# JuliaGaussianProcesses/AugmentedGPLikelihoods.jl

Measured on AMD Instinct MI355X. Metric: CAVI sweeps/sec (N obs, M inducing) + max |Δnat-param| vs CPU ref, higher is better.
Workload: dtype f32 via f16 hi/lo split operands (3 f16 MFMA products per f32 product, f32 accumulate, f64 reductions and M x M update)

## Files before the change

augmentedgplikelihoods.jl_amd/csrc/agpl_syrk.hip:

```cpp
#include <cstdlib>

#include "agpl_common.h"

namespace {

typedef _Float16 h8 __attribute__((ext_vector_type(8)));
typedef float f32x4 __attribute__((ext_vector_type(4)));
typedef unsigned u32x4 __attribute__((ext_vector_type(4)));

constexpr int BS = 128;
constexpr int kPanel = 256;
constexpr int kStagePts = 32;
constexpr uint32_t kImageMagic = 0x41474951u;

struct AccImageHeader {
    uint32_t magic;
    int32_t scale_exp;
    float max_abs;
    uint32_t reserved;
    int64_t N;
    int32_t M;
    int32_t pad[57];
};
static_assert(sizeof(AccImageHeader) == 256, "header size");

__device__ __forceinline__ f32x4 mfma32(h8 a, h8 b, f32x4 c) {
    return __builtin_amdgcn_mfma_f32_16x16x32_f16(a, b, c, 0, 0, 0);
}

#define AGPL_E_SPLIT2(x0_, s0_, x1_, s1_, H_, L_)                                                              \
    do {                                                                                                       \
        asm("v_fma_mixlo_f16 %0, %1, %2, 0" : "=v"(H_) : "v"(x0_), "v"(s0_));                                  \
        asm("v_fma_mixhi_f16 %0, %1, %2, 0" : "+v"(H_) : "v"(x1_), "v"(s1_));                                  \
        asm("v_fma_mixlo_f16 %0, %1, %2, -%3 op_sel_hi:[0,0,1]" : "=v"(L_) : "v"(x0_), "v"(s0_), "v"(H_));     \
        asm("v_fma_mixhi_f16 %0, %1, %2, -%3 op_sel:[0,0,1] op_sel_hi:[0,0,1]"                                 \
            : "+v"(L_)                                                                                         \
            : "v"(x1_), "v"(s1_), "v"(H_));                                                                    \
    } while (0)
#define AGPL_E_GFMA(acc_, b_, x_) asm volatile("v_fmac_f32 %0, %1, %2" : "+v"(acc_) : "v"(b_), "v"(x_))
#define AGPL_Q_JOIN2(H_, L_, x0_, x1_)                                                                         \
    do {                                                                                                       \
        asm("v_fma_mix_f32 %0, %1, 1.0, %2 op_sel_hi:[1,0,1]" : "=v"(x0_) : "v"(H_), "v"(L_));                 \
        asm("v_fma_mix_f32 %0, %1, 1.0, %2 op_sel:[1,0,1] op_sel_hi:[1,0,1]" : "=v"(x1_) : "v"(H_), "v"(L_));  \
    } while (0)

__global__ __launch_bounds__(256) void absmax_kernel(int64_t n4, int ntail, const float4 *__restrict__ x, unsigned *__restrict__ out) {
    unsigned m = 0u;
    for (int64_t i = (int64_t)blockIdx.x * blockDim.x + threadIdx.x; i < n4; i += (int64_t)gridDim.x * blockDim.x) {
        const float4 v = x[i];
        m = max(m, __float_as_uint(v.x) & 0x7FFFFFFFu);
        m = max(m, __float_as_uint(v.y) & 0x7FFFFFFFu);
        m = max(m, __float_as_uint(v.z) & 0x7FFFFFFFu);
        m = max(m, __float_as_uint(v.w) & 0x7FFFFFFFu);
    }
    if (blockIdx.x == 0 && (int)threadIdx.x < ntail)
        m = max(m, __float_as_uint(reinterpret_cast<const float *>(x)[4 * n4 + threadIdx.x]) & 0x7FFFFFFFu);
#pragma unroll
    for (int o = 32; o > 0; o >>= 1) m = max(m, (unsigned)__shfl_xor((int)m, o));
    if ((threadIdx.x & 63) == 0 && m) atomicMax(out, m);
}

__global__ __launch_bounds__(256) void find_bad_kernel(int64_t n, const float *__restrict__ x, float limit,
                                                       unsigned long long *__restrict__ out) {
    for (int64_t i = (int64_t)blockIdx.x * blockDim.x + threadIdx.x; i < n; i += (int64_t)gridDim.x * blockDim.x) {
        const float a = fabsf(x[i]);
        if (!(a < limit)) atomicMin(out, (unsigned long long)i);
    }
}

__global__ __launch_bounds__(256) void accumulate_image_kernel(int64_t N, int M, int Msrc, int64_t nps, float scale, int scale_exp,
                                                               float max_abs, const float *__restrict__ Phi,
                                                               unsigned char *__restrict__ image) {
    __shared__ float tile[16][BS + 1];
    const int nb = M / BS;
    if (blockIdx.x == 0 && threadIdx.x == 0) {
        AccImageHeader *h = reinterpret_cast<AccImageHeader *>(image);
        h->magic = kImageMagic;
        h->scale_exp = scale_exp;
        h->max_abs = max_abs;
        h->reserved = 0;
        h->N = N;
        h->M = M;
    }
    h8 *blocks = reinterpret_cast<h8 *>(image + sizeof(AccImageHeader));
    const int64_t nblk = nps * nb;
    for (int64_t blk = blockIdx.x; blk < nblk; blk += gridDim.x) {
        const int64_t ps = blk / nb;
        const int fb = (int)(blk - ps * nb);
        {
            const int pt = threadIdx.x >> 4, f0 = (threadIdx.x & 15) * 8;
            const int64_t n = ps * 16 + pt;
            float4 a = {0.f, 0.f, 0.f, 0.f}, b = a;
            if (n < N) {
                const int fg = fb * BS + f0;
                const float *src = Phi + n * (int64_t)Msrc + fg;
                if (!(Msrc & 3) && fg + 8 <= Msrc) {
                    a = *reinterpret_cast<const float4 *>(src);
                    b = *reinterpret_cast<const float4 *>(src + 4);
                } else {
                    float t[8];
#pragma unroll
                    for (int j = 0; j < 8; ++j) t[j] = fg + j < Msrc ? src[j] : 0.f;
                    a = float4{t[0], t[1], t[2], t[3]};
                    b = float4{t[4], t[5], t[6], t[7]};
                }
            }
            float *d = &tile[pt][f0];
            d[0] = a.x; d[1] = a.y; d[2] = a.z; d[3] = a.w;
            d[4] = b.x; d[5] = b.y; d[6] = b.z; d[7] = b.w;
        }
        __syncthreads();
        const int plane = threadIdx.x >> 7, row = threadIdx.x & 127;
        h8 hi, lo;
#pragma unroll
        for (int j = 0; j < 8; ++j) {
            const float x = tile[plane * 8 + j][row] * scale;
            const _Float16 a = (_Float16)x;
            hi[j] = a;
            lo[j] = (_Float16)(x - (float)a);
        }
        blocks[(blk * 2 + 0) * 256 + threadIdx.x] = hi;
        blocks[(blk * 2 + 1) * 256 + threadIdx.x] = lo;
        __syncthreads();
    }
}

__global__ __launch_bounds__(256) void acc_prep_kernel(int64_t N, int64_t Npad, int L, const float *__restrict__ gamma,
                                                        const float *__restrict__ beta, float *__restrict__ gb,
                                                        unsigned *__restrict__ scal) {
    __shared__ unsigned red[2][4];
    const int64_t total = (int64_t)L * Npad;
    unsigned m = 0u, bd = 0u;
    for (int64_t i = (int64_t)blockIdx.x * blockDim.x + threadIdx.x; i < total; i += (int64_t)gridDim.x * blockDim.x) {
        const int64_t l = i / Npad, n = i - l * Npad;
        const bool in = n < N;
        const float gv = in ? gamma[l * N + n] : 0.f;
        const unsigned gbits = __float_as_uint(gv), ab = gbits & 0x7FFFFFFFu;
        const bool bad = ab >= 0x7F800000u || ((gbits >> 31) && ab != 0u);
        if (bad) bd = max(bd, (unsigned)min((int64_t)0x7FFFFFFE, l * N + n) + 1u);
        m = max(m, bad ? 0u : ab);
        float *rec = gb + (l * (Npad / 32) + n / 32) * 64 + (n & 31);
        rec[0] = gv;
        rec[32] = in ? beta[l * N + n] : 0.f;
    }
#pragma unroll
    for (int o = 32; o > 0; o >>= 1) {
        m = max(m, (unsigned)__shfl_xor((int)m, o));
        bd = max(bd, (unsigned)__shfl_xor((int)bd, o));
    }
    if ((threadIdx.x & 63) == 0) {
        red[0][threadIdx.x >> 6] = m;
        red[1][threadIdx.x >> 6] = bd;
    }
    __syncthreads();
    if (threadIdx.x == 0) {
        for (int w = 1; w < 4; ++w) {
            m = max(m, red[0][w]);
            bd = max(bd, red[1][w]);
        }
        if (m) atomicMax(scal, m);
        if (bd) atomicMax(scal + 1, bd);
    }
}

__device__ __forceinline__ int acc_scale_exp(unsigned gmax) {
    int eB = gmax ? 126 - (int)(gmax >> 23) : 0;
    return eB < -60 ? -60 : (eB > 60 ? 60 : eB);
}

#ifdef AGPL_QTRACE
__device__ unsigned long long g_qtrace[64 * 16 * 8];
constexpr bool kTrace = true;
#else
constexpr bool kTrace = false;
#endif

#ifdef AGPL_SYRK_L2PROBE
#define AGPL_PROBE_T(t_) ((t_) & 3)
#else
#define AGPL_PROBE_T(t_) (t_)
#endif
#ifdef AGPL_SYRK_NODMA
#define AGPL_PROBE_LOAD(t_) ((t_) < 3)
#else
#define AGPL_PROBE_LOAD(t_) true
#endif
#ifndef AGPL_S_PRE
#define AGPL_S_PRE 3
#endif
constexpr int kStepBytes = 32768;
constexpr int kRing = 4;
constexpr int kRecBytes = 256;
constexpr int kStripLds = kRing * kStepBytes + 8 * kRing * kRecBytes;

template <bool DIAG>
__device__ __forceinline__ void syrk_strip_body(unsigned char *smem_raw, int64_t N, int64_t Npad, int M, int nsplit, int chunk, int nbig, int small, int l,
                                                int s, int I, int J, const unsigned char *__restrict__ image,
                                                const float *__restrict__ gb_all, const unsigned *__restrict__ scal,
                                                float *__restrict__ slabG, float *__restrict__ slabg) {
    typedef __attribute__((address_space(3))) void lds_void;
    const int lane = threadIdx.x & 63;
    const int wave = __builtin_amdgcn_readfirstlane(threadIdx.x >> 6);
    const int nb = M / BS;
    const int cq0 = DIAG ? wave : 2 * wave, cq1 = DIAG ? 15 - wave : 2 * wave + 1;
    const AccImageHeader *hdr = reinterpret_cast<const AccImageHeader *>(image);
    const h8 *blocks = reinterpret_cast<const h8 *>(image + sizeof(AccImageHeader));
    const int eA = hdr->scale_exp;
    const int eB = acc_scale_exp(scal[0]);
    const float sB = __uint_as_float((unsigned)(127 + eB) << 23);

    int64_t nbeg, nend;
    agpl_slice_range(s, chunk, nbig, small, N, nbeg, nend);
    const int nstep = (int)((nend - nbeg + kStagePts - 1) / kStagePts);
    const int64_t ps0 = nbeg / 16;
    const int64_t slice_pitch = (int64_t)nb * 2 * 256;

    int ln = lane;
    asm volatile("" : "+v"(ln));
    const int kg = ln >> 4, lr = ln & 15;
    const int rbS = (wave >> 2) & 1, qd = wave & 3;
    const h8 *a_src = blocks + ((ps0 * nb + 2 * I + rbS) * 2) * 256 + qd * 64 + lane;
    const int a_dst = rbS * 2 * 4096 + qd * 1024;
    const int R0 = 32 * wave + lr;
    const h8 *b_src = blocks + (((ps0 + (kg >> 1)) * nb + 2 * J + (R0 >> 7)) * 2) * 256 + (kg & 1) * 128 + (R0 & 127);
    const float *gb_src = gb_all + ((int64_t)l * (Npad / 32) + nbeg / 32) * 64 + lane;
    float *gbuf = reinterpret_cast<float *>(smem_raw + kRing * kStepBytes + wave * kRing * kRecBytes);

    f32x4 acc[16][2];
#pragma unroll
    for (int i = 0; i < 16; ++i) acc[i][0] = acc[i][1] = f32x4{0.f, 0.f, 0.f, 0.f};
    float gacc0 = 0.f, gacc1 = 0.f;
    u32x4 rh0 = {0, 0, 0, 0}, rl0 = rh0, rh1 = rh0, rl1 = rh0;
    h8 bh0, bl0, bh1, bl1;

#define AGPL_S_DMA(t_, k_)                     \
    do {                                                                                                        \
        unsigned char *d_ = smem_raw + ((t_) & (kRing - 1)) * kStepBytes + ((k_) >> 1) * 16384 + a_dst + ((k_) & 1) * 4096; \
        const h8 *src_ = a_src + (int64_t)(2 * AGPL_PROBE_T(t_) + ((k_) >> 1)) * slice_pitch + ((k_) & 1) * 256; \
        if (AGPL_PROBE_LOAD(t_)) __builtin_amdgcn_global_load_lds(src_, (lds_void *)d_, 16, 0, 0);              \
    } while (0)
#define AGPL_S_DMAG(t_)                                                                                         \
    if (AGPL_PROBE_LOAD(t_))                                                                                    \
    __builtin_amdgcn_global_load_lds(gb_src + (int64_t)(t_) * 64, (lds_void *)(gbuf + ((t_) & (kRing - 1)) * 64), 4, 0, 0)
#define AGPL_S_LOADB(t_)                                                                                        \
    do {                                                                                                        \
        const h8 *src_ = b_src + (int64_t)(2 * AGPL_PROBE_T(t_)) * slice_pitch;                                 \
        const h8 *srcl_ = src_ + 256;  \
        if (AGPL_PROBE_LOAD(t_))                                                                                \
        asm volatile("global_load_dwordx4 %0, %4, off\n\tglobal_load_dwordx4 %1, %5, off\n\t"                   \
                     "global_load_dwordx4 %2, %4, off offset:256\n\tglobal_load_dwordx4 %3, %5, off offset:256"  \
                     : "+v"(rh0), "+v"(rl0), "+v"(rh1), "+v"(rl1)                                               \
                     : "v"(src_), "v"(srcl_)                                                                    \
                     : "memory");                                                                               \
    } while (0)
#define AGPL_S_CVT(RH_, RL_, g0_, g1_, b0_, b1_, GA_)                                                           \
    do {                                                                                                        \
        float x0_, x1_;                                                                                         \
        AGPL_Q_JOIN2(RH_, RL_, x0_, x1_);                                                                       \
        if (DIAG) {                                                                                             \
            AGPL_E_GFMA(GA_, b0_, x0_);                                                                         \
            AGPL_E_GFMA(GA_, b1_, x1_);                                                                         \
        }                                                                                                       \
        AGPL_E_SPLIT2(x0_, g0_, x1_, g1_, RH_, RL_);                                                            \
    } while (0)
#define AGPL_S_CVTQ(q_, tt_, keepf_)                                                                            \
    do {                                                                                                        \
        const float *gq_ = gbuf + ((tt_) & (kRing - 1)) * 64 + 8 * kg + 4 * ((q_) & 1);                         \
        float4 g4_ = *reinterpret_cast<const float4 *>(gq_);                                                    \
        g4_.x *= sB, g4_.y *= sB, g4_.z *= sB, g4_.w *= sB;                                                     \
        float4 b4_ = {0.f, 0.f, 0.f, 0.f};                                                                      \
        if (DIAG) {                                                                                             \
            b4_ = *reinterpret_cast<const float4 *>(gq_ + 32);                                                  \
            if (!(keepf_)) b4_ = float4{0.f, 0.f, 0.f, 0.f};                                                    \
        }                                                                                                       \
        if ((q_) == 0) {                                                                                        \
            AGPL_S_CVT(rh0.x, rl0.x, g4_.x, g4_.y, b4_.x, b4_.y, gacc0);                                        \
            AGPL_S_CVT(rh0.y, rl0.y, g4_.z, g4_.w, b4_.z, b4_.w, gacc0);                                        \
            AGPL_S_CVT(rh1.x, rl1.x, g4_.x, g4_.y, b4_.x, b4_.y, gacc1);                                        \
            AGPL_S_CVT(rh1.y, rl1.y, g4_.z, g4_.w, b4_.z, b4_.w, gacc1);                                        \
        } else {                                                                                                \
            AGPL_S_CVT(rh0.z, rl0.z, g4_.x, g4_.y, b4_.x, b4_.y, gacc0);                                        \
            AGPL_S_CVT(rh0.w, rl0.w, g4_.z, g4_.w, b4_.z, b4_.w, gacc0);                                        \
            AGPL_S_CVT(rh1.z, rl1.z, g4_.x, g4_.y, b4_.x, b4_.y, gacc1);                                        \
            AGPL_S_CVT(rh1.w, rl1.w, g4_.z, g4_.w, b4_.z, b4_.w, gacc1);                                        \
        }                                                                                                       \
    } while (0)
#define AGPL_S_TAKEB()                       \
    do {                                                                                                        \
        bh0 = __builtin_bit_cast(h8, rh0);                                                                      \
        bl0 = __builtin_bit_cast(h8, rl0);                                                                      \
        bh1 = __builtin_bit_cast(h8, rh1);                                                                      \
        bl1 = __builtin_bit_cast(h8, rl1);                                                                      \
    } while (0)

    const int fa = (kg >> 1) * 1024 + (kg & 1) * 128 + lr;
#define AGPL_S_AOFF(i_) (fa + ((i_) >> 3) * 512 + ((i_) & 7) * 16)
#define AGPL_S_LDSB(t_)                                                                                         \
    do {                                                                                                        \
        const u32x4 *sn_ = reinterpret_cast<const u32x4 *>(smem_raw + ((t_) & (kRing - 1)) * kStepBytes);       \
        rh0 = sn_[AGPL_S_AOFF(cq0)];                                                                            \
        rl0 = sn_[256 + AGPL_S_AOFF(cq0)];                                                                      \
        rh1 = sn_[AGPL_S_AOFF(cq1)];                                                                            \
        rl1 = sn_[256 + AGPL_S_AOFF(cq1)];                                                                      \
    } while (0)

#pragma unroll
    for (int t = 0; t < 3; ++t)
        if (t < nstep) {
            AGPL_S_DMAG(t);
            AGPL_S_DMA(t, 0);
            AGPL_S_DMA(t, 1);
            AGPL_S_DMA(t, 2);
            AGPL_S_DMA(t, 3);
        }
    if (!DIAG) AGPL_S_LOADB(0);
    asm volatile("s_waitcnt vmcnt(0)" ::: "memory");
    __builtin_amdgcn_sched_barrier(0);
    if (DIAG) {
        __builtin_amdgcn_s_barrier();
        AGPL_S_LDSB(0);
    }
    AGPL_S_CVTQ(0, 0, true);
    AGPL_S_CVTQ(1, 0, true);
    AGPL_S_TAKEB();
    if (!DIAG) AGPL_S_LOADB(nstep > 1 ? 1 : 0);

    [[maybe_unused]] unsigned long long q0 = 0, q1 = 0, qw = 0, qa = 0, qb = 0, qr0 = 0;
    if (kTrace) {
        q0 = __builtin_amdgcn_s_memtime();
        qr0 = __builtin_amdgcn_s_memrealtime();
    }
    for (int t = 0; t < nstep; ++t) {
        if (kTrace) qa = __builtin_amdgcn_s_memtime();
        if (!DIAG) __builtin_amdgcn_s_barrier();
        if (kTrace && !DIAG) qw += __builtin_amdgcn_s_memtime() - qa;
        const bool more = t + 1 < nstep;
        const int tl = t + 2 < nstep ? t + 2 : nstep - 1;
        const h8 *st = reinterpret_cast<const h8 *>(smem_raw + (t & (kRing - 1)) * kStepBytes);
#define AGPL_S_HOOK(h_)                                                                                         \
    do {                                                                                                        \
        if (!DIAG) {                                                                                            \
            if ((h_) < 4 && t + 3 < nstep) {                                                                    \
                if ((h_) == 0) AGPL_S_DMAG(t + 3);                                                              \
                AGPL_S_DMA(t + 3, h_);                                                                          \
            }                                                                                                   \
            if ((h_) == 5) {  \
                __builtin_amdgcn_sched_barrier(0);                                                              \
                if (kTrace) qb = __builtin_amdgcn_s_memtime();                                                  \
                if (t + 3 < nstep) asm volatile("s_waitcnt vmcnt(5)" ::: "memory");                             \
                else asm volatile("s_waitcnt vmcnt(0)" ::: "memory");                                           \
                if (kTrace) q1 += __builtin_amdgcn_s_memtime() - qb;                                            \
                __builtin_amdgcn_sched_barrier(0);                                                              \
            }                                                                                                   \
            if ((h_) == 6) AGPL_S_CVTQ(0, t + 1, more);                                                         \
            if ((h_) == 8) AGPL_S_CVTQ(1, t + 1, more);                                                         \
        } else {                                                                                                \
             \
             \
             \
                 \
            if ((h_) == 7) {                                                                                    \
                __builtin_amdgcn_sched_barrier(0);                                                              \
                if (kTrace) qb = __builtin_amdgcn_s_memtime();                                                  \
                if (t + 2 < nstep) asm volatile("s_waitcnt vmcnt(5)" ::: "memory");                             \
                else asm volatile("s_waitcnt vmcnt(0)" ::: "memory");                                           \
                if (kTrace) q1 += __builtin_amdgcn_s_memtime() - qb;                                            \
                if (kTrace) qb = __builtin_amdgcn_s_memtime();                                                  \
                __builtin_amdgcn_s_barrier();                                                                   \
                if (kTrace) qw += __builtin_amdgcn_s_memtime() - qb;                                            \
                __builtin_amdgcn_sched_barrier(0);                                                              \
                AGPL_S_LDSB(more ? t + 1 : t);                 \
            }                                                                                                   \
            if ((h_) >= 8 && (h_) < 12 && t + 3 < nstep) {                                                      \
                if ((h_) == 8) AGPL_S_DMAG(t + 3);                                                              \
                AGPL_S_DMA(t + 3, (h_) - 8);                                                                    \
            }                                                                                                   \
            if ((h_) == 9) AGPL_S_CVTQ(0, t + 1, more);                                                         \
            if ((h_) == 11) AGPL_S_CVTQ(1, t + 1, more);                                                        \
        }                                                                                                       \
    } while (0)
        h8 nbh0, nbl0, nbh1, nbl1;
        constexpr int kPre = AGPL_S_PRE;
        h8 af[kPre + 1][2];
#pragma unroll
        for (int j = 0; j < kPre; ++j) {
            af[j][0] = st[AGPL_S_AOFF(j)];
            af[j][1] = st[256 + AGPL_S_AOFF(j)];
        }
#pragma unroll
        for (int i = 0; i < 16; ++i) {
            if (!DIAG && (i == 0 || i == 12)) {
                if ((wave >= 4) == (i == 0)) __builtin_amdgcn_s_setprio(1);
                else __builtin_amdgcn_s_setprio(0);
            }
            if (i + kPre < 16) {
                af[(i + kPre) % (kPre + 1)][0] = st[AGPL_S_AOFF(i + kPre)];
                af[(i + kPre) % (kPre + 1)][1] = st[256 + AGPL_S_AOFF(i + kPre)];
            }
            if (!DIAG) {
                const h8 ahc = af[i % (kPre + 1)][0], alc = af[i % (kPre + 1)][1];
                acc[i][0] = mfma32(ahc, bh0, acc[i][0]);
                acc[i][1] = mfma32(ahc, bh1, acc[i][1]);
                acc[i][0] = mfma32(ahc, bl0, acc[i][0]);
                acc[i][1] = mfma32(ahc, bl1, acc[i][1]);
                acc[i][0] = mfma32(alc, bh0, acc[i][0]);
                acc[i][1] = mfma32(alc, bh1, acc[i][1]);
            } else {
                const h8 ahc = af[i % (kPre + 1)][0], alc = af[i % (kPre + 1)][1];
                if (i >= cq0) {
                    acc[i][0] = mfma32(ahc, bh0, acc[i][0]);
                    acc[i][0] = mfma32(ahc, bl0, acc[i][0]);
                    acc[i][0] = mfma32(alc, bh0, acc[i][0]);
                }
                if (i >= cq1) {
                    acc[i][1] = mfma32(ahc, bh1, acc[i][1]);
                    acc[i][1] = mfma32(ahc, bl1, acc[i][1]);
                    acc[i][1] = mfma32(alc, bh1, acc[i][1]);
                }
            }
            AGPL_S_HOOK(i);
            if (i == (DIAG ? 12 : 10)) {
                nbh0 = __builtin_bit_cast(h8, rh0);
                nbl0 = __builtin_bit_cast(h8, rl0);
                nbh1 = __builtin_bit_cast(h8, rh1);
                nbl1 = __builtin_bit_cast(h8, rl1);
                if (!DIAG) AGPL_S_LOADB(tl);
            }
        }
#undef AGPL_S_HOOK
        bh0 = nbh0;
        bl0 = nbl0;
        bh1 = nbh1;
        bl1 = nbl1;
    }
    if (!DIAG) __builtin_amdgcn_s_setprio(0);
#ifdef AGPL_QTRACE
    if (blockIdx.x < 64 && lane == 0) {
        unsigned long long *o = g_qtrace + ((size_t)blockIdx.x * 16 + wave) * 8;
        o[0] = q1;
        o[1] = __builtin_amdgcn_s_memtime() - q0;
        o[2] = qw;
        o[5] = __builtin_amdgcn_s_memrealtime() - qr0;
        o[6] = (unsigned long long)nstep | ((unsigned long long)(DIAG ? 1 : 0) << 32) | ((unsigned long long)cq0 << 40);
        o[7] = o[1];
    }
#endif
    asm volatile("s_waitcnt vmcnt(0)" ::: "memory");
    asm volatile("" ::"v"(rh0), "v"(rl0), "v"(rh1), "v"(rl1));
#undef AGPL_S_DMA
#undef AGPL_S_DMAG
#undef AGPL_S_LOADB
#undef AGPL_S_CVT
#undef AGPL_S_CVTQ
#undef AGPL_S_TAKEB
#undef AGPL_S_LDSB
#undef AGPL_S_AOFF

    const float unscale = __uint_as_float((unsigned)(127 - (2 * eA + eB)) << 23);
    const int npairs = nb * (nb + 1) / 2;
#pragma unroll
    for (int hb = 0; hb < 2; ++hb) {
        const int bi = 2 * I + hb;
#pragma unroll
        for (int cb = 0; cb < 2; ++cb) {
            const int q = cb ? cq1 : cq0;
            const int bj = 2 * J + (q >> 3);
            if (DIAG && bi < bj) continue;
            const int p128 = bi * (bi + 1) / 2 + bj;
            float *slab = slabG + (((int64_t)l * npairs + p128) * nsplit + s) * (int64_t)(BS * BS);
#pragma unroll
            for (int ii = 0; ii < 8; ++ii)
#pragma unroll
                for (int r = 0; r < 4; ++r) {
                    const int row = 16 * ii + 4 * kg + r;
                    const int col = (q & 7) * 16 + lr;
                    slab[row * BS + col] = acc[8 * hb + ii][cb][r] * unscale;
                }
        }
    }
    if (DIAG) {
        gacc0 += __shfl_xor(gacc0, 16);
        gacc0 += __shfl_xor(gacc0, 32);
        gacc1 += __shfl_xor(gacc1, 16);
        gacc1 += __shfl_xor(gacc1, 32);
        const float g1s = __shfl(gacc1, (lane - 16) & 63);
        if (lane < 32) {
            const int rr = 16 * (lane < 16 ? cq0 : cq1) + (lane & 15);
            slabg[(((int64_t)l * nb + 2 * I + (rr >> 7)) * nsplit + s) * BS + (rr & 127)] =
                (lane < 16 ? gacc0 : g1s) * __uint_as_float((unsigned)(127 - eA) << 23);
        }
    }
}


__global__ __launch_bounds__(512, 2) void syrk_strip_kernel(int64_t N, int64_t Npad, int M, int nlat, int npairs2, int nsplit, int chunk, int nbig, int small,
                                                            const unsigned char *__restrict__ image,
                                                            const float *__restrict__ gb_all,
                                                            const unsigned *__restrict__ scal,
                                                            float *__restrict__ slabG, float *__restrict__ slabg) {
    extern __shared__ __attribute__((aligned(16))) unsigned char smem_raw[];
    const int id = blockIdx.x;
    const int xcd = id & 7, jj = id >> 3;
    const int per_s = nlat * npairs2;
    const int s = (jj / per_s) * 8 + xcd;
    const int rem = jj % per_s;
    const int l = rem / npairs2;
    const int p2 = rem - l * npairs2;
    if (s >= nsplit) return;
    const int nb2 = M / kPanel;
    const int noff = nb2 * (nb2 - 1) / 2;
    int I, J;
    if (p2 < noff) {
        I = 1;
        while ((I + 1) * I / 2 <= p2) ++I;
        J = p2 - I * (I - 1) / 2;
    } else {
        I = J = p2 - noff;
    }
    if (I == J) syrk_strip_body<true>(smem_raw, N, Npad, M, nsplit, chunk, nbig, small, l, s, I, J, image, gb_all, scal, slabG, slabg);
    else syrk_strip_body<false>(smem_raw, N, Npad, M, nsplit, chunk, nbig, small, l, s, I, J, image, gb_all, scal, slabG, slabg);
}

}

#ifdef AGPL_QTRACE
extern "C" __attribute__((visibility("default"))) int agpl_debug_qtrace(unsigned long long *out) {
    return (int)hipMemcpyFromSymbol(out, HIP_SYMBOL(g_qtrace), sizeof(g_qtrace));
}
#endif


static_assert(sizeof(AccImageHeader) == 256 && BS == 128 && kStagePts == 32,
              "agpl_accumulate_image_bytes (agpl_common.h) assumes this layout");

int32_t agpl_feature_range_check(agpl_ctx *ctx, int64_t N, int32_t M, const float *Phi, float limit, const char *what,
                                 unsigned *max_bits_out) {
    int32_t rc = agpl_ws2_reserve(ctx, 4096);
    if (rc) return rc;
    if ((uintptr_t)Phi & 15) AGPL_FAIL(ctx, AGPL_ERR_INVALID_ARGUMENT, "the feature matrix must be 16-byte aligned");
    unsigned *mx = (unsigned *)ctx->ws2 + 512;
    AGPL_HIP(ctx, hipMemsetAsync(mx, 0, 16, ctx->stream));
    const int64_t n = N * (int64_t)M, n4 = n / 4;
    absmax_kernel<<<4096, 256, 0, ctx->stream>>>(n4, (int)(n - 4 * n4), reinterpret_cast<const float4 *>(Phi), mx);
    AGPL_LAUNCH_CHECK(ctx);
    unsigned hmx = 0, hlim;
    memcpy(&hlim, &limit, 4);
    AGPL_HIP(ctx, hipMemcpyAsync(&hmx, mx, sizeof(unsigned), hipMemcpyDeviceToHost, ctx->stream));
    AGPL_HIP(ctx, hipStreamSynchronize(ctx->stream));
    if (hmx >= 0x7F800000u || hmx >= hlim) {
        unsigned long long *bad = (unsigned long long *)(mx + 2), hbad = ~0ull;
        AGPL_HIP(ctx, hipMemsetAsync(bad, 0xFF, 8, ctx->stream));
        find_bad_kernel<<<4096, 256, 0, ctx->stream>>>(n, Phi, limit, bad);
        AGPL_HIP(ctx, hipMemcpyAsync(&hbad, bad, 8, hipMemcpyDeviceToHost, ctx->stream));
        AGPL_HIP(ctx, hipStreamSynchronize(ctx->stream));
        const long long pt = (long long)(hbad / (unsigned long long)M), ft = (long long)(hbad % (unsigned long long)M);
        if (hmx >= 0x7F800000u && !(limit < __builtin_inff()))
            AGPL_FAIL(ctx, AGPL_ERR_DOMAIN, "feature value is not finite (point %lld, feature %lld)", pt, ft);
        AGPL_FAIL(ctx, AGPL_ERR_DOMAIN,
                  "feature value is not finite or its magnitude is not below %g, the range of %s (point %lld, feature %lld)",
                  (double)limit, what, pt, ft);
    }
    *max_bits_out = hmx;
    return AGPL_OK;
}

int32_t agpl_image_scale_exp(agpl_ctx *ctx, unsigned hmx, int *eA_out) {
    int eA = 0;
    if (hmx) {
        const int ex = (int)(hmx >> 23) - 127;
        eA = 13 - ex;
        if (eA > 37 || eA < -30) {
            float mx;
            memcpy(&mx, &hmx, 4);
            AGPL_FAIL(ctx, AGPL_ERR_DOMAIN,
                      "max |Phi| = %g is outside the range the split-float16 images can be scaled for (2^-24 .. 2^44): rescale the "
                      "features", (double)mx);
        }
        if (eA > 30) eA = 30;
    }
    *eA_out = eA;
    return AGPL_OK;
}
int32_t agpl_accumulate_image_build(agpl_ctx *ctx, int64_t N, int32_t M, int32_t Msrc, const float *Phi, int eA, unsigned hmx,
                                    void *image_out) {
    float max_abs;
    memcpy(&max_abs, &hmx, 4);
    const float scale = ldexpf(1.f, eA);
    const int64_t nps = ((N + kStagePts - 1) / kStagePts) * 2;
    accumulate_image_kernel<<<16384, 256, 0, ctx->stream>>>(N, M, Msrc, nps, scale, eA, max_abs, Phi, (unsigned char *)image_out);
    AGPL_LAUNCH_CHECK(ctx);
    if (ctx->checked_image == image_out) ctx->checked_image = nullptr;
    return AGPL_OK;
}

int32_t agpl_syrk_image_launch(agpl_ctx *ctx, int64_t N, int64_t Npad, int32_t M, int32_t L, const void *image,
                               const float *gamma, const float *beta, float *gb, unsigned *scal, float *slabG,
                               float *slabg, int ns, int chunk, int nbig, int small, bool records_ready) {
    if (M % kPanel) AGPL_FAIL(ctx, AGPL_ERR_INVALID_ARGUMENT, "the image accumulation needs M %% 256 == 0 (M = %d)", M);
    if (ctx->checked_image != image || ctx->checked_image_N != N || ctx->checked_image_M != M) {
        AccImageHeader h;
        AGPL_HIP(ctx, hipMemcpyAsync(&h, image, sizeof(h), hipMemcpyDeviceToHost, ctx->stream));
        AGPL_HIP(ctx, hipStreamSynchronize(ctx->stream));
        if (h.magic != kImageMagic || h.N != N || h.M != M)
            AGPL_FAIL(ctx, AGPL_ERR_INVALID_ARGUMENT,
                      "not an accumulate image of this problem (agpl_plan_create): header says N = %lld, "
                      "M = %d, magic %#x; the call has N = %lld, M = %d",
                      (long long)h.N, (int)h.M, (unsigned)h.magic, (long long)N, (int)M);
        ctx->checked_image = image;
        ctx->checked_image_N = N;
        ctx->checked_image_M = M;
    }
    const int nb2 = M / kPanel;
    const int npairs2 = nb2 * (nb2 + 1) / 2;
    const int64_t nwg = (int64_t)L * npairs2 * ((ns + 7) / 8) * 8;
    if (nwg > 0x7fffffffLL) AGPL_FAIL(ctx, AGPL_ERR_INVALID_ARGUMENT, "problem too large for one launch");
    if (!records_ready) {
        AGPL_HIP(ctx, hipMemsetAsync(scal, 0, 2 * sizeof(unsigned), ctx->stream));
        int64_t nblk = agpl_cdiv((int64_t)L * Npad, 256);
        if (nblk > 1024) nblk = 1024;
        acc_prep_kernel<<<(unsigned)nblk, 256, 0, ctx->stream>>>(N, Npad, L, gamma, beta, gb, scal);
        AGPL_LAUNCH_CHECK(ctx);
    }
    if (!ctx->strip_attr) {
        AGPL_HIP(ctx, hipFuncSetAttribute(reinterpret_cast<const void *>(&syrk_strip_kernel),
                                          hipFuncAttributeMaxDynamicSharedMemorySize, kStripLds));
        ctx->strip_attr = 1;
    }
    syrk_strip_kernel<<<(unsigned)nwg, 512, kStripLds, ctx->stream>>>(N, Npad, M, L, npairs2, ns, chunk, nbig, small, (const unsigned char *)image, gb,
                                                                     scal, slabG, slabg);
    AGPL_LAUNCH_CHECK(ctx);
    return AGPL_OK;
}
```

Before: 77.46.

## Specialize diagonal SYRK strip per wave and place prefetch hooks by MFMA work

Diagonal SYRK strips are now compiled as eight per-wave template instances with a compile-time wave index. Each wave's i-loop starts at its first active column block, which skips the empty leading iterations. The prefetch, convert and barrier hooks are scheduled by the cumulative count of MFMA triples instead of the loop index, so memory work spreads evenly over the compute each wave actually does. The diagonal t-loop is unrolled by two, the final-step waitcnt is simplified using clamped prefetch indices, and an optional LDS-wait trace is added. The cost is code size and instruction-cache pressure from eight body copies, plus redundant clamped loads on the last steps.

```diff
diff --git a/augmentedgplikelihoods.jl_amd/csrc/agpl_syrk.hip b/augmentedgplikelihoods.jl_amd/csrc/agpl_syrk.hip
--- a/augmentedgplikelihoods.jl_amd/csrc/agpl_syrk.hip
+++ b/augmentedgplikelihoods.jl_amd/csrc/agpl_syrk.hip
@@ -171,8 +171,10 @@
 #ifdef AGPL_QTRACE
 __device__ unsigned long long g_qtrace[64 * 16 * 8];
 constexpr bool kTrace = true;
+constexpr bool kTraceLds = AGPL_QTRACE + 0 >= 2;
 #else
 constexpr bool kTrace = false;
+constexpr bool kTraceLds = false;
 #endif
 
 #ifdef AGPL_SYRK_L2PROBE
@@ -193,16 +195,20 @@
 constexpr int kRecBytes = 256;
 constexpr int kStripLds = kRing * kStepBytes + 8 * kRing * kRecBytes;
 
-template <bool DIAG>
+constexpr int diag_triples(int W, int i) { return i < W ? 0 : (i - W + 1) + (i >= 15 - W ? i - (15 - W) + 1 : 0); }
+static_assert(diag_triples(0, 15) == 17 && diag_triples(7, 15) == 17 && diag_triples(7, 7) == 1 && diag_triples(3, 2) == 0, "");
+
+template <bool DIAG, int W>
 __device__ __forceinline__ void syrk_strip_body(unsigned char *smem_raw, int64_t N, int64_t Npad, int M, int nsplit, int chunk, int nbig, int small, int l,
                                                 int s, int I, int J, const unsigned char *__restrict__ image,
                                                 const float *__restrict__ gb_all, const unsigned *__restrict__ scal,
                                                 float *__restrict__ slabG, float *__restrict__ slabg) {
     typedef __attribute__((address_space(3))) void lds_void;
     const int lane = threadIdx.x & 63;
-    const int wave = __builtin_amdgcn_readfirstlane(threadIdx.x >> 6);
+    const int wave = DIAG ? W : __builtin_amdgcn_readfirstlane(threadIdx.x >> 6);
     const int nb = M / BS;
-    const int cq0 = DIAG ? wave : 2 * wave, cq1 = DIAG ? 15 - wave : 2 * wave + 1;
+    const int cq0 = DIAG ? W : 2 * wave, cq1 = DIAG ? 15 - W : 2 * wave + 1;
+    constexpr int i0 = DIAG ? W : 0;
     const AccImageHeader *hdr = reinterpret_cast<const AccImageHeader *>(image);
     const h8 *blocks = reinterpret_cast<const h8 *>(image + sizeof(AccImageHeader));
     const int eA = hdr->scale_exp;
@@ -233,15 +239,17 @@
     u32x4 rh0 = {0, 0, 0, 0}, rl0 = rh0, rh1 = rh0, rl1 = rh0;
     h8 bh0, bl0, bh1, bl1;
 
-#define AGPL_S_DMA(t_, k_)                     \
+#define AGPL_S_DMAX(t_, ts_, k_)                                                                                \
     do {                                                                                                        \
         unsigned char *d_ = smem_raw + ((t_) & (kRing - 1)) * kStepBytes + ((k_) >> 1) * 16384 + a_dst + ((k_) & 1) * 4096; \
-        const h8 *src_ = a_src + (int64_t)(2 * AGPL_PROBE_T(t_) + ((k_) >> 1)) * slice_pitch + ((k_) & 1) * 256; \
+        const h8 *src_ = a_src + (int64_t)(2 * AGPL_PROBE_T(ts_) + ((k_) >> 1)) * slice_pitch + ((k_) & 1) * 256; \
         if (AGPL_PROBE_LOAD(t_)) __builtin_amdgcn_global_load_lds(src_, (lds_void *)d_, 16, 0, 0);              \
     } while (0)
-#define AGPL_S_DMAG(t_)                                                                                         \
+#define AGPL_S_DMA(t_, k_) AGPL_S_DMAX(t_, t_, k_)
+#define AGPL_S_DMAGX(t_, ts_)                                                                                   \
     if (AGPL_PROBE_LOAD(t_))                                                                                    \
-    __builtin_amdgcn_global_load_lds(gb_src + (int64_t)(t_) * 64, (lds_void *)(gbuf + ((t_) & (kRing - 1)) * 64), 4, 0, 0)
+    __builtin_amdgcn_global_load_lds(gb_src + (int64_t)(ts_) * 64, (lds_void *)(gbuf + ((t_) & (kRing - 1)) * 64), 4, 0, 0)
+#define AGPL_S_DMAG(t_) AGPL_S_DMAGX(t_, t_)
 #define AGPL_S_LOADB(t_)                                                                                        \
     do {                                                                                                        \
         const h8 *src_ = b_src + (int64_t)(2 * AGPL_PROBE_T(t_)) * slice_pitch;                                 \
@@ -325,18 +333,20 @@
     AGPL_S_TAKEB();
     if (!DIAG) AGPL_S_LOADB(nstep > 1 ? 1 : 0);
 
-    [[maybe_unused]] unsigned long long q0 = 0, q1 = 0, qw = 0, qa = 0, qb = 0, qr0 = 0;
+    [[maybe_unused]] unsigned long long q0 = 0, q1 = 0, qw = 0, qa = 0, qb = 0, qr0 = 0, ql = 0, qc = 0;
     if (kTrace) {
         q0 = __builtin_amdgcn_s_memtime();
         qr0 = __builtin_amdgcn_s_memrealtime();
     }
-    for (int t = 0; t < nstep; ++t) {
+    auto step = [&](const int t) __attribute__((always_inline)) {
         if (kTrace) qa = __builtin_amdgcn_s_memtime();
         if (!DIAG) __builtin_amdgcn_s_barrier();
         if (kTrace && !DIAG) qw += __builtin_amdgcn_s_memtime() - qa;
         const bool more = t + 1 < nstep;
         const int tl = t + 2 < nstep ? t + 2 : nstep - 1;
+        [[maybe_unused]] const int td = t + 3 < nstep ? t + 3 : nstep - 1;
         const h8 *st = reinterpret_cast<const h8 *>(smem_raw + (t & (kRing - 1)) * kStepBytes);
+#define AGPL_S_AT(n_) (diag_triples(W, i) >= (n_) && diag_triples(W, i - 1) < (n_))
 #define AGPL_S_HOOK(h_)                                                                                         \
     do {                                                                                                        \
         if (!DIAG) {                                                                                            \
@@ -358,12 +368,15 @@
              \
              \
              \
-                 \
-            if ((h_) == 7) {                                                                                    \
+             \
+             \
+             \
+             \
+             \
+            if (AGPL_S_AT(8)) {                                                                                  \
                 __builtin_amdgcn_sched_barrier(0);                                                              \
                 if (kTrace) qb = __builtin_amdgcn_s_memtime();                                                  \
-                if (t + 2 < nstep) asm volatile("s_waitcnt vmcnt(5)" ::: "memory");                             \
-                else asm volatile("s_waitcnt vmcnt(0)" ::: "memory");                                           \
+                asm volatile("s_waitcnt vmcnt(5)" ::: "memory");                                                \
                 if (kTrace) q1 += __builtin_amdgcn_s_memtime() - qb;                                            \
                 if (kTrace) qb = __builtin_amdgcn_s_memtime();                                                  \
                 __builtin_amdgcn_s_barrier();                                                                   \
@@ -371,28 +384,42 @@
                 __builtin_amdgcn_sched_barrier(0);                                                              \
                 AGPL_S_LDSB(more ? t + 1 : t);                 \
             }                                                                                                   \
-            if ((h_) >= 8 && (h_) < 12 && t + 3 < nstep) {                                                      \
-                if ((h_) == 8) AGPL_S_DMAG(t + 3);                                                              \
-                AGPL_S_DMA(t + 3, (h_) - 8);                                                                    \
+            if (AGPL_S_AT(9)) {                                                                                 \
+                AGPL_S_DMAGX(t + 3, td);                                                                        \
+                AGPL_S_DMAX(t + 3, td, 0);                                                                      \
             }                                                                                                   \
-            if ((h_) == 9) AGPL_S_CVTQ(0, t + 1, more);                                                         \
-            if ((h_) == 11) AGPL_S_CVTQ(1, t + 1, more);                                                        \
+            if (AGPL_S_AT(10)) AGPL_S_DMAX(t + 3, td, 1);                                                       \
+            if (AGPL_S_AT(11)) AGPL_S_DMAX(t + 3, td, 2);                                                       \
+            if (AGPL_S_AT(12)) AGPL_S_DMAX(t + 3, td, 3);                                                       \
+            if (AGPL_S_AT(10)) AGPL_S_CVTQ(0, t + 1, more);                                                     \
+            if (AGPL_S_AT(12)) AGPL_S_CVTQ(1, t + 1, more);                                                     \
         }                                                                                                       \
+    } while (0)
+#define AGPL_S_LDSSTAMP(sum_)              \
+    do {                                                                                                        \
+        __builtin_amdgcn_sched_barrier(0);                                                                      \
+        qb = __builtin_amdgcn_s_memtime();                                                                      \
+        asm volatile("s_waitcnt lgkmcnt(0)" ::: "memory");                                                      \
+        sum_ += __builtin_amdgcn_s_memtime() - qb;                                                              \
+        asm volatile("s_waitcnt lgkmcnt(0)" ::: "memory");                                                      \
+        __builtin_amdgcn_sched_barrier(0);                                                                      \
     } while (0)
         h8 nbh0, nbl0, nbh1, nbl1;
         constexpr int kPre = AGPL_S_PRE;
+        static_assert(kPre >= 1 && 7 + kPre <= 16, "the lead of the fragment reads");
         h8 af[kPre + 1][2];
 #pragma unroll
-        for (int j = 0; j < kPre; ++j) {
-            af[j][0] = st[AGPL_S_AOFF(j)];
-            af[j][1] = st[256 + AGPL_S_AOFF(j)];
-        }
-#pragma unroll
-        for (int i = 0; i < 16; ++i) {
+        for (int j = i0; j < i0 + kPre; ++j) {
+            af[j % (kPre + 1)][0] = st[AGPL_S_AOFF(j)];
+            af[j % (kPre + 1)][1] = st[256 + AGPL_S_AOFF(j)];
+        }
+#pragma unroll
+        for (int i = i0; i < 16; ++i) {
             if (!DIAG && (i == 0 || i == 12)) {
                 if ((wave >= 4) == (i == 0)) __builtin_amdgcn_s_setprio(1);
                 else __builtin_amdgcn_s_setprio(0);
             }
+            if (kTraceLds && DIAG) AGPL_S_LDSSTAMP(ql);
             if (i + kPre < 16) {
                 af[(i + kPre) % (kPre + 1)][0] = st[AGPL_S_AOFF(i + kPre)];
                 af[(i + kPre) % (kPre + 1)][1] = st[256 + AGPL_S_AOFF(i + kPre)];
@@ -419,7 +446,7 @@
                 }
             }
             AGPL_S_HOOK(i);
-            if (i == (DIAG ? 12 : 10)) {
+            if (DIAG ? AGPL_S_AT(13) : i == 10) {
                 nbh0 = __builtin_bit_cast(h8, rh0);
                 nbl0 = __builtin_bit_cast(h8, rl0);
                 nbh1 = __builtin_bit_cast(h8, rh1);
@@ -428,10 +455,22 @@
             }
         }
 #undef AGPL_S_HOOK
+#undef AGPL_S_AT
+        if (kTraceLds && DIAG) AGPL_S_LDSSTAMP(qc);
+#undef AGPL_S_LDSSTAMP
         bh0 = nbh0;
         bl0 = nbl0;
         bh1 = nbh1;
         bl1 = nbl1;
+    };
+    if (DIAG) {
+        for (int t = 0; t < nstep; t += 2) {
+            step(t);
+            if (t + 1 >= nstep) break;
+            step(t + 1);
+        }
+    } else {
+        for (int t = 0; t < nstep; ++t) step(t);
     }
     if (!DIAG) __builtin_amdgcn_s_setprio(0);
 #ifdef AGPL_QTRACE
@@ -440,8 +479,11 @@
         o[0] = q1;
         o[1] = __builtin_amdgcn_s_memtime() - q0;
         o[2] = qw;
+        o[3] = ql;
+        o[4] = qc;
         o[5] = __builtin_amdgcn_s_memrealtime() - qr0;
-        o[6] = (unsigned long long)nstep | ((unsigned long long)(DIAG ? 1 : 0) << 32) | ((unsigned long long)cq0 << 40);
+        o[6] = (unsigned long long)nstep | ((unsigned long long)(DIAG ? 1 : 0) << 32) | ((unsigned long long)cq0 << 40) |
+               ((unsigned long long)(kTraceLds && DIAG ? 16 - i0 : 0) << 48);
         o[7] = o[1];
     }
 #endif
@@ -449,6 +491,8 @@
     asm volatile("" ::"v"(rh0), "v"(rl0), "v"(rh1), "v"(rl1));
 #undef AGPL_S_DMA
 #undef AGPL_S_DMAG
+#undef AGPL_S_DMAX
+#undef AGPL_S_DMAGX
 #undef AGPL_S_LOADB
 #undef AGPL_S_CVT
 #undef AGPL_S_CVTQ
@@ -517,8 +561,23 @@
     } else {
         I = J = p2 - noff;
     }
-    if (I == J) syrk_strip_body<true>(smem_raw, N, Npad, M, nsplit, chunk, nbig, small, l, s, I, J, image, gb_all, scal, slabG, slabg);
-    else syrk_strip_body<false>(smem_raw, N, Npad, M, nsplit, chunk, nbig, small, l, s, I, J, image, gb_all, scal, slabG, slabg);
+#define AGPL_S_BODY(DIAG_, W_) \
+    syrk_strip_body<DIAG_, W_>(smem_raw, N, Npad, M, nsplit, chunk, nbig, small, l, s, I, J, image, gb_all, scal, slabG, slabg)
+    if (I == J) {
+        switch (__builtin_amdgcn_readfirstlane(threadIdx.x >> 6)) {
+        case 0: AGPL_S_BODY(true, 0); break;
+        case 1: AGPL_S_BODY(true, 1); break;
+        case 2: AGPL_S_BODY(true, 2); break;
+        case 3: AGPL_S_BODY(true, 3); break;
+        case 4: AGPL_S_BODY(true, 4); break;
+        case 5: AGPL_S_BODY(true, 5); break;
+        case 6: AGPL_S_BODY(true, 6); break;
+        default: AGPL_S_BODY(true, 7); break;
+        }
+    } else {
+        AGPL_S_BODY(false, 0);
+    }
+#undef AGPL_S_BODY
 }
 
 }
```

New measurement: 76.02. 0.981x the previous value.
